# CZY-Code/PHNet

Measured on AMD Instinct MI355X. Metric: clips/s (5x3x320x800) fwd+bwd, higher is better.
Workload: dtype f32 storage / accumulation, every product as an EXACT three-term bf16 split (6 bf16 MFMAs, f32-MFMA accuracy); 1 GPU; 5-frame clip 3x320x800, resnet34 + router + lane head, fwd+bwd+AdamW, 1 clip/GPU/step, random-init weights; parallelism=dp1, launch=hipGraph replay of the whole step

## Files before the change

include/phnet_hip.h:

```cpp
#ifndef PHNET_HIP_H
#define PHNET_HIP_H
#include <stdint.h>
#ifdef __cplusplus
extern "C" {
#endif

#define PHNET_OK 0
#define PHNET_ERR_ARG (-1)
#define PHNET_ERR_WORKSPACE (-2)
#define PHNET_ERR_LAUNCH (-3)
#define PHNET_ABI_VERSION 1

int phnet_abi_version(void);

int phnet_lane_nms(const float* rows, const float* scores, const int32_t* counts, int64_t frames,
                   int64_t k_max, int32_t n_offsets, float thresh, int64_t top_k,
                   int64_t* keep, int64_t* num_to_keep, int64_t* parent, void* stream);

int phnet_lane_decode(const float* lines, int64_t frames, int32_t N, int32_t n_offsets, float conf_thresh,
                      float nms_thresh, int64_t top_k, float img_w, uint8_t* keep_mask, int64_t* num,
                      int64_t* keep_c, int64_t* anchors, int64_t* anchors_sorted, float* kept_rows, void* stream);

int phnet_lane_points(const float* kept_rows, const int64_t* num, const float* prior_ys, int64_t F, int32_t L, int32_t S,
                      float* points, int32_t* count, int32_t* lanes_num, int32_t* slot, void* stream);

int phnet_lane_track(const float* kept_rows, const int64_t* num, int64_t B, int32_t T, int32_t L, int32_t S, int32_t M, float thr,
                     int32_t max_age, int32_t* trk_id, int32_t* trk_missed, int32_t* trk_hits, int32_t* trk_ext, float* trk_x,
                     int32_t* next_id, int32_t* track_id, int32_t* track_hits, void* stream);

int phnet_lane_draw(const float* points, const int32_t* count, const int32_t* lanes_num, const int32_t* slot,
                    const int32_t* track_id, int64_t F, int32_t L, int32_t S, double sx, double sy, double oy,
                    int32_t out_h, int32_t out_w, int32_t lane_width, const uint8_t* src, int32_t src_format,
                    int64_t frame_stride, int32_t pitch, int64_t chroma_offset, const int32_t* csc_host,
                    const uint8_t* palette, int32_t alpha, uint8_t* label_map, uint8_t* overlay, void* stream);

int phnet_lane_targets(const float* points, const int32_t* counts, const int32_t* lanes_num, const double* offsets_ys, float* out,
                       int64_t F, int32_t Lin, int32_t P, int32_t R, int32_t S, double img_h, double img_w, double strip_size,
                       double crop, double src_w, double scale_x, double scale_y, int32_t flip, void* stream);
int phnet_lane_targets_aug(const float* points, const int32_t* counts, const int32_t* lanes_num, const double* offsets_ys, float* out,
                           int64_t F, int32_t Lin, int32_t P, int32_t R, int32_t S, double img_h, double img_w, double strip_size,
                           double crop, double src_w, double scale_x, double scale_y, int32_t flip, const int32_t* flip2,
                           const double* fwd, void* stream);
int phnet_lane_targets_clip(const float* points, const int32_t* counts, const int32_t* lanes_num, const double* offsets_ys, float* out,
                            int64_t F, int32_t Lin, int32_t P, int32_t R, int32_t S, double img_h, double img_w, double strip_size,
                            double crop, double src_w, double scale_x, double scale_y, int32_t flip, const int32_t* flip2,
                            const double* fwd, int32_t clip, int32_t* frag_count, void* stream);

int phnet_roi_pool_fwd(const float* fmap, const float* xs, const float* ys, float* out, float* out_cp,
                       int32_t B, int32_t N, int32_t P, int32_t h, int32_t w, int32_t C, void* stream);
int phnet_roi_pool_bwd(const float* dout, const float* fmap, const float* xs, const float* ys,
                       float* dmap, float* dxs,
                       int32_t B, int32_t N, int32_t P, int32_t h, int32_t w, int32_t C, void* stream);

int phnet_conv2d_fwd(const float* x, const float* w, const float* bias, float* y,
                     int32_t N, int32_t Hi, int32_t Wi, int32_t Ci, int32_t Co, int32_t R, int32_t S,
                     int32_t stride, int32_t pad, int32_t relu, void* workspace, uint64_t ws_bytes, void* stream);
uint64_t phnet_conv2d_stats_blocks(int64_t M, int32_t Co, int32_t K, uint64_t ws_bytes);
int phnet_conv2d_fwd_fused(const float* x, const float* w, const float* bias, const float* addend, float* y, float* stats,
                           int32_t N, int32_t Hi, int32_t Wi, int32_t Ci, int32_t Co, int32_t R, int32_t S,
                           int32_t stride, int32_t pad, int32_t relu, void* workspace, uint64_t ws_bytes, void* stream);
int phnet_conv2d_dgrad(const float* dy, const float* w, const float* addend, float* dx,
                       int32_t N, int32_t Hi, int32_t Wi, int32_t Ci, int32_t Co, int32_t R, int32_t S,
                       int32_t stride, int32_t pad, void* workspace, uint64_t ws_bytes, void* stream);
int phnet_conv3p_applies(int64_t M, int32_t Ca, int32_t Nn);
uint64_t phnet_conv3p_packed_bytes(int32_t Co, int32_t Ci);
int phnet_conv3p_pack(const float* w, void* packed, int32_t Co, int32_t Ci, int32_t dgrad, void* stream);
int phnet_conv3p_pack_jobs(const void* jobs, int32_t njobs, int64_t total, void* stream);
uint64_t phnet_conv3p_stats_blocks(int64_t M, int32_t Ca, int32_t Nn, uint64_t ws_bytes);
int phnet_conv3p_fwd(const float* x, const void* packed, const float* bias, const float* addend, float* y, float* stats,
                     int32_t N, int32_t H, int32_t W, int32_t Ca, int32_t Nn, int32_t relu,
                     void* workspace, uint64_t ws_bytes, void* stream);
int phnet_conv2d_plan(int64_t M, int32_t Co, int32_t K, uint64_t ws_bytes, int32_t* bm, int32_t* bn, int32_t* splits,
                      int32_t* k_tile);
int phnet_conv2d_kernel(int32_t dgrad, int32_t N, int32_t Hi, int32_t Wi, int32_t Ci, int32_t Co, int32_t R, int32_t S,
                        int32_t stride, int32_t pad, uint64_t ws_bytes, char* name, int32_t name_cap, int32_t* splits);
int phnet_conv2d_wgrad_kernel(int32_t N, int32_t Hi, int32_t Wi, int32_t Ci, int32_t Co, int32_t R, int32_t S, int32_t stride,
                              int32_t pad, int32_t has_dbias, uint64_t ws_bytes, char* name, int32_t name_cap, int32_t* splits);
int phnet_linear_bwd_kernel(int32_t M, int32_t K, int32_t N, int32_t has_relu_mask, char* name, int32_t name_cap);
int phnet_conv3p_kernel(int64_t M, int32_t Ca, int32_t Nn, uint64_t ws_bytes, char* name, int32_t name_cap, int32_t* splits);
uint64_t phnet_conv2d_wgrad_workspace(int32_t N, int32_t Hi, int32_t Wi, int32_t Ci, int32_t Co,
                                      int32_t R, int32_t S, int32_t stride, int32_t pad);
int phnet_conv2d_wgrad(const float* dy, const float* x, float* dw, float* dbias,
                       int32_t N, int32_t Hi, int32_t Wi, int32_t Ci, int32_t Co, int32_t R, int32_t S,
                       int32_t stride, int32_t pad, int32_t accumulate, void* workspace, uint64_t ws_bytes, void* stream);
int phnet_linear_bwd_fusable(int64_t M, int64_t K, int64_t N);
int phnet_linear_bwd(const float* dy, const float* x, const float* w, const float* relu_y, float* dx, float* dw, float* dbias,
                     int32_t M, int32_t K, int32_t N, int32_t accumulate, void* stream);
int phnet_nchw3_to_nhwc4(const float* x, float* y, int32_t N, int32_t H, int32_t W, void* stream);
int phnet_pad_channels(const float* src, float* dst, int64_t rows, int32_t cs, int32_t cd, void* stream);

uint64_t phnet_ipc_buffer_bytes(int32_t world, uint64_t max_bytes);
int phnet_ipc_alloc(uint64_t bytes, void** ptr);
int phnet_ipc_free(void* ptr);
int phnet_ipc_get_handle(void* ptr, void* handle64);
int phnet_ipc_open_handle(const void* handle64, void** ptr);
int phnet_ipc_close_handle(void* ptr);
int phnet_oneshot_allreduce(void* data, int32_t count, int32_t dtype, const void* peers, int32_t rank, int32_t world,
                            int32_t cap, void* ctrl, void* stream);

uint64_t phnet_channel_partials_size(int64_t M, int32_t C);
int phnet_bn_fwd_stats(const float* x, int64_t M, int32_t C, float eps, float momentum,
                       const float* gamma, const float* beta, float* running_mean, float* running_var,
                       float* save_mean, float* save_invstd, float* scale, float* shift,
                       float* partial, int32_t training, void* stream);
int phnet_bn_finalize_partials(const float* partial, int64_t nblk, int64_t M, int32_t C, float eps, float momentum,
                               const float* gamma, const float* beta, float* running_mean, float* running_var,
                               float* save_mean, float* save_invstd, float* scale, float* shift, void* stream);
int phnet_bn_apply(const float* x, const float* scale, const float* shift, const float* residual, float* y,
                   int64_t M, int32_t C, int32_t relu, void* stream);
int phnet_bn_bwd(const float* dy, const float* x, const float* y, const float* save_mean,
                 const float* save_invstd, const float* gamma, float* dx, float* dres,
                 float* dgamma, float* dbeta, float* partial, float* c1, float* c2,
                 int64_t M, int32_t C, int32_t relu, int32_t dres_accumulate, int32_t param_accumulate, void* stream);

int phnet_bn_bwd_reduce(const float* dy, const float* x, const float* y, const float* mean, const float* invstd,
                        float* sums, float* partial, float* c1_scratch, float* c2_scratch,
                        int64_t M, int32_t C, int32_t relu, void* stream);
int phnet_bn_bwd_apply(const float* dy, const float* x, const float* y, const float* mean, const float* invstd,
                       const float* gamma, const float* c1, const float* c2, float* dx, float* dres,
                       int64_t M, int32_t C, int32_t relu, int32_t dres_accumulate, void* stream);

int phnet_bn_local_sums(const float* x, int64_t M, int32_t C, float* partial, double* sums, void* stream);
int phnet_bn_partials_to_sums(const float* partial, int64_t nblk, int64_t M, int32_t C, double* sums, void* stream);
int phnet_bn_finalize_sums(const double* sums, int32_t C, float eps, float momentum, const float* gamma, const float* beta,
                           float* running_mean, float* running_var, float* save_mean, float* save_invstd,
                           float* scale, float* shift, void* stream);
int phnet_bn_bwd_apply_sums(const float* dy, const float* x, const float* y, const float* mean, const float* invstd,
                            const float* gamma, const float* sums, const double* count, float* c1, float* c2,
                            float* dx, float* dres, int64_t M, int32_t C, int32_t relu, int32_t dres_accumulate, void* stream);

int phnet_preprocess_u8(const uint8_t* frames, float* out, uint8_t* out_u8,
                        const int32_t* xi, const int16_t* xc, const int32_t* yi, const int16_t* yc,
                        int32_t T, int32_t H0, int32_t W0, int32_t crop_top, int32_t out_h, int32_t out_w, int32_t flip,
                        int32_t layout, const float* mean3_host, const float* std3_host, void* stream);
int phnet_preprocess_yuv(const uint8_t* frames, float* out, uint8_t* out_u8,
                         const int32_t* xi, const int16_t* xc, const int32_t* yi, const int16_t* yc,
                         int32_t T, int32_t H0, int32_t W0, int32_t crop_top, int32_t out_h, int32_t out_w, int32_t flip, int32_t layout,
                         int32_t format, int64_t frame_stride, int32_t pitch, int64_t chroma_offset,
                         const int32_t* csc_host, const float* mean3_host, const float* std3_host, void* stream);

int phnet_augment_u8(const uint8_t* frames, float* out, uint8_t* out_u8, const int32_t* flip2, const double* inv, const int32_t* table,
                     int32_t T, int32_t H, int32_t W, int32_t layout, const float* mean3_host, const float* std3_host, void* stream);

int phnet_augment_stencil_u8(const uint8_t* frames, float* out, uint8_t* out_u8, const int32_t* flip2, const double* inv,
                             const int32_t* table, const int32_t* stencil, uint8_t* staged, int32_t T, int32_t H, int32_t W, int32_t layout,
                             const float* mean3_host, const float* std3_host, void* stream);

int phnet_lane_raster(const int32_t* segs, int64_t n_segs, uint32_t* masks, int32_t n_lanes, int32_t height, int32_t width,
                      int32_t lane_width, void* stream);
int phnet_lane_mask_stats(const uint32_t* masks, int32_t n_lanes, int32_t height, int32_t width, const int32_t* pairs,
                          int32_t n_pairs, int64_t* area, int64_t* inter, void* stream);
int phnet_lane_iou_groups(const uint32_t* masks, int32_t n_lanes, int32_t height, int32_t width, const int32_t* groups,
                          int32_t n_groups, int64_t n_entries, int32_t scale, double eps, double* iou, int64_t* area,
                          void* stream);
// ... 199 lines not shown
```

phnet_amd/build.py:

```python
import glob
import os
import subprocess
import sys

HERE = os.path.dirname(os.path.abspath(__file__))
CSRC = os.path.join(HERE, "csrc")
OBJ = os.path.join(HERE, "lib", "obj")
SO = os.path.join(HERE, "lib", "libphnet_hip.so")
FLAGS = ["--offload-arch=gfx950", "-O3", "-std=c++17", "-fPIC", "-fvisibility=hidden", "-Wall", "-Wno-unused-function"]
EXTRA_FLAGS = {"wgrad3s.hip": ["-fno-slp-vectorize"], "wgrad1s.hip": ["-fno-slp-vectorize"]}


def _hipcc():
    for c in (os.environ.get("HIPCC"), "/opt/rocm/bin/hipcc", "hipcc"):
        if c and (os.path.isabs(c) and os.path.exists(c) or not os.path.isabs(c)):
            return c
    raise RuntimeError("hipcc not found")


def build(force: bool = False, verbose: bool = True) -> str:
    os.makedirs(OBJ, exist_ok=True)
    srcs = sorted(glob.glob(os.path.join(CSRC, "*.hip")))
    hdrs = glob.glob(os.path.join(CSRC, "*.h")) + [os.path.join(os.path.dirname(HERE), "include", "phnet_hip.h")]
    newest_hdr = max([os.path.getmtime(h) for h in hdrs] + [0.0])
    objs, procs = [], []
    for s in srcs:
        o = os.path.join(OBJ, os.path.basename(s)[:-4] + ".o")
        objs.append(o)
        if force or not os.path.exists(o) or os.path.getmtime(o) < max(os.path.getmtime(s), newest_hdr):
            if verbose:
                print("[phnet_amd.build] hipcc", os.path.basename(s), flush=True)
            procs.append((s, subprocess.Popen([_hipcc(), *FLAGS, *EXTRA_FLAGS.get(os.path.basename(s), []), "-c", s, "-o", o])))
    for s, p in procs:
        if p.wait() != 0:
            raise RuntimeError(f"hipcc failed on {s}")
    if procs or not os.path.exists(SO) or any(os.path.getmtime(o) > os.path.getmtime(SO) for o in objs):
        subprocess.check_call([_hipcc(), "--offload-arch=gfx950", "-shared", "-fPIC", "-o", SO, *objs])
    return SO


if __name__ == "__main__":
    print(build(force="--force" in sys.argv))
```

phnet_amd/csrc/conv.hip:

```cpp
#include <cstdio>
#include "conv_igemm.h"
#include "tuning.h"

using namespace igemm;

namespace {

constexpr int T3_AROWS = 66;
template <bool DGRAD>
__global__ __launch_bounds__(THREADS) void conv3x3s1_kernel(
    const float* __restrict__ X, const float* __restrict__ Wt, const float* __restrict__ bias,
    const float* __restrict__ addend, float* __restrict__ out, ConvShape g, int relu, float* __restrict__ stats)
{
    constexpr int APITCH = KContigPlanes<64, 16>::PITCH;
    constexpr int APLANE = T3_AROWS * APITCH, AIMG = 3 * APLANE;
    typedef KContigPlanes<64, 16> BP3C;
    typedef KStridedPlanes<64, 16> BP3S;
    constexpr int BIMG = DGRAD ? BP3S::BYTES : BP3C::BYTES;
    constexpr int BPLANE = DGRAD ? BP3S::PLANE : BP3C::PLANE;
    extern __shared__ __attribute__((aligned(16))) float lds[];
    unsigned char* A3 = reinterpret_cast<unsigned char*>(lds);
    unsigned char* B3 = A3 + 2 * AIMG;
    unsigned char* dump = B3 + 2 * BIMG;

    const int W = g.Wi, H = g.Hi, Ca = g.Ci;
    const int M = g.N * H * W, K = 9 * Ca;
    const int CC = Ca >> 4;
    const int tiles_n = (g.Co + 63) >> 6;
    const unsigned tile = xcd_remap(blockIdx.x, gridDim.x);
    const int m0 = (int)(tile / tiles_n) * 64, n0 = (int)(tile % tiles_n) * 64;
    const int u_begin = blockIdx.z * g.k_per_split, u_end = min(3 * CC, u_begin + g.k_per_split);
    const int tid = threadIdx.x, lane = tid & 63, wave = tid >> 6;
    const int wm = (wave >> 1) * 32, wn = (wave & 1) * 32;

    constexpr unsigned OOB = 0x80000000u;
    __amdgpu_buffer_rsrc_t x_rsrc = __builtin_amdgcn_make_buffer_rsrc((void*)X, 0, (int)min((long)M * Ca * 4, (long)0x7fffffff), 0x00020000);
    __amdgpu_buffer_rsrc_t w_rsrc = __builtin_amdgcn_make_buffer_rsrc((void*)Wt, 0, (int)min((long)g.Co * K * 4, (long)0x7fffffff), 0x00020000);
    int a_off[2], a_ok[2], a_lds[2];
#pragma unroll
    for (int i = 0; i < 2; ++i) {
        const int idx = tid + 256 * i, row = idx >> 2, chunk = idx & 3;
        const bool rowok = idx < 4 * T3_AROWS;
        const int t = m0 - 1 + row;
        const bool tok = rowok && (unsigned)t < (unsigned)M;
        const int tt = tok ? t : 0;
        const int y = (tt / W) % H;
        a_ok[i] = (tok && y >= 1 ? 1 : 0) | (tok ? 2 : 0) | (tok && y + 1 < H ? 4 : 0);
        a_off[i] = (t * Ca + chunk * 4) * 4;
        a_lds[i] = rowok ? row * APITCH + chunk * 8 : -1;
    }
    const int a_row = tid >> 2, a_chunk = tid & 3;
    const int b_kk = tid >> 4, b_ch = tid & 15;
    int b_off, b_lds;
    if (!DGRAD) {
        const int n = n0 + a_row;
        b_off = n < g.Co ? (n * K + a_chunk * 4) * 4 : (int)OOB;
        b_lds = a_row * BP3C::PITCH + a_chunk * 8;
    } else {
        const int n = n0 + b_ch * 4;
        b_off = n < g.Co ? (b_kk * 9 * g.Co + n) * 4 : (int)OOB;
        b_lds = b_kk * BP3S::PITCH + b_ch * 8;
    }
    int la_dy = u_begin / CC, la_cc = u_begin - la_dy * CC, la_u = u_begin;
    int lb_dy = la_dy, lb_cc = la_cc, lb_u = u_begin, lb_dx = 0;
    const bool wave0 = __builtin_amdgcn_readfirstlane(wave) == 0;
    auto load_a = [&](f32x4 (&reg)[2]) {
        const bool uok = la_u < u_end;
        const int s_a = ((la_dy - 1) * W * Ca + la_cc * 16) * 4;
        {
            const bool ok = uok && ((a_ok[0] >> la_dy) & 1);
            reg[0] = __builtin_bit_cast(f32x4, __builtin_amdgcn_raw_buffer_load_b128(x_rsrc, ok ? a_off[0] + s_a : (int)OOB, 0, 0));
        }
        if (wave0) {
            const bool ok = uok && ((a_ok[1] >> la_dy) & 1);
            reg[1] = __builtin_bit_cast(f32x4, __builtin_amdgcn_raw_buffer_load_b128(x_rsrc, ok ? a_off[1] + s_a : (int)OOB, 0, 0));
        }
        ++la_u; ++la_cc;
        const int wrap = la_cc == CC;
        la_cc = wrap ? 0 : la_cc;
        la_dy += wrap;
    };
    auto load_b = [&](f32x4& reg) {
        const bool uok = lb_u < u_end;
        const int s_b = !DGRAD ? ((lb_dy * 3 + lb_dx) * Ca + lb_cc * 16) * 4
                               : ((lb_cc * 16 * 3 + (2 - lb_dy)) * 3 + (2 - lb_dx)) * g.Co * 4;
// ... 195 lines not shown
    const int mma = tuning().mma_mode;
    if (mma == 3 && M <= 2048) return {64, 64};
    if (mma >= 1) {
        if (N >= 128 && ceil_div64(M, 128) * ceil_div64(N, 128) >= 300) return {128, 128};
        if (ceil_div64(M, 128) * ceil_div64(N, 64) >= 1250) return {128, 64};
    }
    return {64, 64};
}

struct ConvPlan { int bm, bn, splits; long tiles; };

int k_tile_for(long M, int K, int ci, int bm, int bn)
{
    const int mma = tuning().mma_mode;
    if (M <= (mma == 3 ? 256 : 2048) && K >= 64) return (mma == 3 && tuning().deep_kt3 == 32) ? 32 : 64;
    if (mma == 3) return BK;
    if (mma >= 1 && bm == 64 && bn == 64 && ci % 32 == 0) return 32;
    return BK;
}

ConvPlan plan_conv(long M, int Co, int K, bool has_ws, size_t ws_bytes)
{
    const Tuning& tn = tuning();
    TileChoice t = pick_tile(M, Co);
    if (tn.force_bm) {
        t = {tn.force_bm, tn.force_bn};
        ConvPlan f{t.bm, t.bn, 1, ceil_div64(M, t.bm) * ceil_div64(Co, t.bn)};
        int splits = tn.force_splits > 0 ? tn.force_splits : 1;
        while (splits > 1 && (!has_ws || (size_t)splits * M * Co * sizeof(float) > ws_bytes)) --splits;
        f.splits = splits;
        return f;
    }
    ConvPlan p{t.bm, t.bn, 1, ceil_div64(M, t.bm) * ceil_div64(Co, t.bn)};
    const bool deep = M <= (tn.mma_mode == 3 ? 256 : 2048) && K >= 64;
    if (has_ws && p.tiles < (deep ? 400 : 900)) {
        int splits = (int)min((long)8, max((long)1, (1250 + p.tiles / 2) / p.tiles));
        while (splits > 1 && K / splits < 256) --splits;
        while (splits > 1 && (size_t)splits * M * Co * sizeof(float) > ws_bytes) --splits;
        p.splits = splits;
    }
    return p;
}

ConvPick pick_conv(const ConvShape& g, bool dgrad, bool has_ws, size_t ws_bytes)
{
    const Tuning& tn = tuning();
    const long M = (long)g.N * g.Ho * g.Wo;
    const int K = g.R * g.S * g.Ci;
    const ConvPlan t = plan_conv(M, g.Co, K, has_ws, ws_bytes);
    ConvPick p{};
    p.dgrad = dgrad; p.bm = t.bm; p.bn = t.bn; p.splits = t.splits; p.tiles = t.tiles;
    p.bkt = tn.force_kt ? tn.force_kt : k_tile_for(M, K, g.Ci, t.bm, t.bn);
    p.mma = tn.mma_mode;
    p.pf = p.mma == 3 ? ((tn.pf == 4 || tn.pf == 2) ? tn.pf : 1) : (p.mma == 0 && tn.pf == 4) ? 4 : 1;
    const bool uni = (g.Ci % p.bkt) == 0 && tn.uniform_tap;
    p.uni = uni && t.bm == 64 && t.bn == 64;
    p.buf = p.uni && g.in_dil == 1 && tn.buf_loads && p.mma == 3;
    p.taps3 = tn.taps3 && p.buf && g.R == 3 && g.S == 3 && g.stride == 1 && g.pad == 1 && g.Ho == g.Hi && g.Wo == g.Wi &&
              p.bkt == 16 && p.pf == 4 && g.Wi >= 2 && M * (long)g.Ci * 4 < 0x7fffffffL && (long)g.Co * K * 4 < 0x7fffffffL;
    return p;
}

int conv_kernel_name(const ConvPick& p, char* name, int cap)
{
    static const char* const tf[2] = {"false", "true"};
    const int n = p.taps3 ? snprintf(name, (size_t)cap, "conv3x3s1_kernel<%s>", tf[p.dgrad])
                          : snprintf(name, (size_t)cap, "conv_igemm_kernel<%d, %d, %s, %d, %s, %d, %d, %s>", p.bm, p.bn, tf[p.dgrad], p.bkt,
                                     tf[p.uni], p.mma, p.pf, tf[p.buf]);
    return n < cap ? PHNET_OK : PHNET_ERR_ARG;
}

#define PHNET_LAUNCH_CONV___(DGRAD_, BM_, BN_, BKT_, UNI_, PF_)                                                         \
    do {                                                                                                                \
        if (p.buf) PHNET_LAUNCH_CONV____(DGRAD_, BM_, BN_, BKT_, UNI_, 3, PF_, UNI_);                                   \
        else PHNET_LAUNCH_CONV____(DGRAD_, BM_, BN_, BKT_, UNI_, 3, PF_, false);                                        \
    } while (0)
#define PHNET_LAUNCH_CONV_(DGRAD_, BM_, BN_, BKT_, UNI_)                                                                \
    do {                                                                                                                \
        if (p.pf == 4) PHNET_LAUNCH_CONV___(DGRAD_, BM_, BN_, BKT_, UNI_, 4);                                           \
        else if (p.pf == 2) PHNET_LAUNCH_CONV___(DGRAD_, BM_, BN_, BKT_, UNI_, 2);                                      \
        else PHNET_LAUNCH_CONV___(DGRAD_, BM_, BN_, BKT_, UNI_, 1);                                                     \
    } while (0)

template <bool DGRAD>
int launch_conv(const float* X, const float* W, const float* bias, const float* addend, float* out, float* workspace,
                size_t ws_bytes, ConvShape g, int relu, hipStream_t st, float* stats = nullptr)
{
    const ConvPick p = pick_conv(g, DGRAD, workspace != nullptr, ws_bytes);
    const long M = (long)g.N * g.Ho * g.Wo;
    const int K = g.R * g.S * g.Ci;
    const int splits = p.splits;
    g.splits = splits;
    float* dst = splits > 1 ? workspace : out;
    dim3 grid((unsigned)p.tiles, 1, (unsigned)splits);
    const int ksteps = (K + p.bkt - 1) / p.bkt;
    g.k_per_split = ((ksteps + splits - 1) / splits) * p.bkt;
    if (p.taps3) {
        const int units = 3 * (g.Ci / 16);
        g.k_per_split = (units + splits - 1) / splits;
        constexpr size_t lds_ = 2 * 3 * T3_AROWS * KContigPlanes<64, 16>::PITCH +
                                2 * (size_t)(DGRAD ? KStridedPlanes<64, 16>::BYTES : KContigPlanes<64, 16>::BYTES) + 3 * 512;
        hipLaunchKernelGGL((conv3x3s1_kernel<DGRAD>), grid, dim3(THREADS), lds_, st,
                           X, W, bias, addend, dst, g, relu, splits > 1 ? (float*)nullptr : stats);
    } else {
        const ConvLaunch a{X, W, bias, addend, dst, splits > 1 ? (float*)nullptr : stats, &g, relu, grid, st};
        if (p.mma != 3) launch_conv_alt(p, a);
        else PHNET_LAUNCH_CONV_TILES(DGRAD);
    }
    if (splits > 1) {
        const long total4 = M * g.Co / 4;
        hipLaunchKernelGGL(splitk_reduce_kernel, dim3((unsigned)ceil_div64(total4, 256)), dim3(256), 0, st,
                           workspace, out, bias, addend, total4, g.Co, splits, relu, 0, stats);
    }
    return phnet_launch_status();
}

}

PHNET_API int phnet_conv2d_plan(int64_t M, int32_t Co, int32_t K, uint64_t ws_bytes, int32_t* bm, int32_t* bn, int32_t* splits,
                                int32_t* k_tile)
{
    ConvShape g;
    if (M < 1 || M > 0x7fffffffL || Co < 1 || K < 1 || !bm || !bn || !splits || !k_tile) return PHNET_ERR_ARG;
    fwd_shape((int)M, 1, 1, K, Co, 1, 1, 1, 0, &g);
    const ConvPick p = pick_conv(g, false, ws_bytes > 0, (size_t)ws_bytes);
    *bm = p.bm; *bn = p.bn; *splits = p.splits; *k_tile = p.bkt;
    return PHNET_OK;
}

PHNET_API int phnet_conv2d_kernel(int32_t dgrad, int32_t N, int32_t Hi, int32_t Wi, int32_t Ci, int32_t Co, int32_t R, int32_t S,
                                  int32_t stride, int32_t pad, uint64_t ws_bytes, char* name, int32_t name_cap, int32_t* splits)
{
    ConvShape g;
    if (!conv_args_ok(N, Hi, Wi, Ci, Co, R, S, stride, pad) || N < 1 || !name || name_cap < 1 || !splits) return PHNET_ERR_ARG;
    if (dgrad ? (stride > 2 || !dgrad_shape(N, Hi, Wi, Ci, Co, R, S, stride, pad, &g)) : !fwd_shape(N, Hi, Wi, Ci, Co, R, S, stride, pad, &g))
        return PHNET_ERR_ARG;
    const ConvPick p = pick_conv(g, dgrad != 0, ws_bytes > 0, (size_t)ws_bytes);
    *splits = p.splits;
    return conv_kernel_name(p, name, name_cap);
}

PHNET_API int phnet_conv2d_fwd(const float* x, const float* w, const float* bias, float* y,
                               int32_t N, int32_t Hi, int32_t Wi, int32_t Ci, int32_t Co, int32_t R, int32_t S,
                               int32_t stride, int32_t pad, int32_t relu,
                               void* workspace, uint64_t ws_bytes, void* stream)
{
    ConvShape g;
    if (!conv_args_ok(N, Hi, Wi, Ci, Co, R, S, stride, pad)) return PHNET_ERR_ARG;
    if (N == 0) return PHNET_OK;
    if (!x || !w || !y || !fwd_shape(N, Hi, Wi, Ci, Co, R, S, stride, pad, &g)) return PHNET_ERR_ARG;
    return launch_conv<false>(x, w, bias, nullptr, y, (float*)workspace, ws_bytes, g, relu, (hipStream_t)stream);
}

static long conv_stats_blocks(long M, int Co, int K, bool has_ws, size_t ws_bytes)
{
    const ConvPlan t = plan_conv(M, Co, K, has_ws, ws_bytes);
    return t.splits > 1 ? ceil_div64(M * Co / 4, 256) : t.tiles / ceil_div64(Co, t.bn) * (t.bm / 32);
}

PHNET_API uint64_t phnet_conv2d_stats_blocks(int64_t M, int32_t Co, int32_t K, uint64_t ws_bytes)
{
    if (M < 1 || Co < 4 || K < 1) return 0;
    return (uint64_t)conv_stats_blocks((long)M, Co, K, ws_bytes > 0, (size_t)ws_bytes);
}

PHNET_API int phnet_conv2d_fwd_fused(const float* x, const float* w, const float* bias, const float* addend, float* y, float* stats,
                                     int32_t N, int32_t Hi, int32_t Wi, int32_t Ci, int32_t Co, int32_t R, int32_t S,
                                     int32_t stride, int32_t pad, int32_t relu,
                                     void* workspace, uint64_t ws_bytes, void* stream)
{
    ConvShape g;
    if (!conv_args_ok(N, Hi, Wi, Ci, Co, R, S, stride, pad)) return PHNET_ERR_ARG;
    if (stats && (bias || addend || relu || (Co & (Co - 1)) || Co > 1024)) return PHNET_ERR_ARG;
    if (N == 0) return PHNET_OK;
    if (!x || !w || !y || !fwd_shape(N, Hi, Wi, Ci, Co, R, S, stride, pad, &g)) return PHNET_ERR_ARG;
    return launch_conv<false>(x, w, bias, addend, y, (float*)workspace, ws_bytes, g, relu, (hipStream_t)stream, stats);
}

PHNET_API int phnet_conv2d_dgrad(const float* dy, const float* w, const float* addend, float* dx,
                                 int32_t N, int32_t Hi, int32_t Wi, int32_t Ci, int32_t Co, int32_t R, int32_t S,
                                 int32_t stride, int32_t pad, void* workspace, uint64_t ws_bytes, void* stream)
{
    ConvShape g;
    if (!conv_args_ok(N, Hi, Wi, Ci, Co, R, S, stride, pad)) return PHNET_ERR_ARG;
    if (stride > 2) return PHNET_ERR_ARG;
    if (N == 0) return PHNET_OK;
    if (!dy || !w || !dx || !dgrad_shape(N, Hi, Wi, Ci, Co, R, S, stride, pad, &g)) return PHNET_ERR_ARG;
    return launch_conv<true>(dy, w, nullptr, addend, dx, (float*)workspace, ws_bytes, g, 0, (hipStream_t)stream);
}

PHNET_API int phnet_nchw3_to_nhwc4(const float* x, float* y, int32_t N, int32_t H, int32_t W, void* stream)
{
    if (N < 0 || H < 1 || W < 1) return PHNET_ERR_ARG;
    if (N == 0) return PHNET_OK;
    if (!x || !y) return PHNET_ERR_ARG;
    const long total = (long)N * H * W;
    hipLaunchKernelGGL(nchw3_to_nhwc4_kernel, dim3((unsigned)ceil_div64(total, 256)), dim3(256), 0, (hipStream_t)stream,
                       x, y, N, H * W);
    return phnet_launch_status();
}

// ... 10 lines not shown
```

phnet_amd/csrc/tuning.h:

```cpp
#pragma once

struct Tuning {
    int mma_mode = 3;
    int pf = 4;
    int buf_loads = 1;
    int uniform_tap = 1;
    int taps3 = 1;
    int deep_kt3 = 64;
    int force_bm = 0, force_bn = 0, force_splits = 0;
    int force_kt = 0;
    int wgrad_bm128 = 1;
    int wgrad_smallp = 1;
    int wgrad_bkw = 16;
    int wgrad3 = 1;
    int wgrad3_bkw = 16;
    int wgrad3s = 1;
    int wgrad1s = 1;
    int wgrad_target = 768;
    int wgrad3_target = 256;
    int smallp_max_tiles = 400;
    int p3_target = 512;
    int p3_wide = 1;
    int gate_wave = 1;
    int dyn_mfma = 1;
    int dyn_rows = 1;
};

Tuning& tuning();
```

phnet_amd/csrc/tuning.hip:

```cpp
#include "common.h"
#include "tuning.h"

Tuning& tuning() { static Tuning t; return t; }

PHNET_API int phnet_tune_reset(void) { tuning() = Tuning{}; return PHNET_OK; }
PHNET_API int phnet_tune_mma_get(void) { return tuning().mma_mode; }

PHNET_API int phnet_tune_force_conv_tile(int32_t bm, int32_t bn, int32_t splits)
{
    if (bm != 0 && !((bm == 64 || bm == 128) && (bn == 64 || bn == 128))) return PHNET_ERR_ARG;
    Tuning& t = tuning();
    t.force_bm = bm; t.force_bn = bn; t.force_splits = splits;
    return PHNET_OK;
}

PHNET_API int phnet_tune_force_k_tile(int32_t kt)
{
    Tuning& t = tuning();
    if (kt == -1 || kt == -2) { t.uniform_tap = kt == -2; return PHNET_OK; }
    if (kt == -5 || kt == -6) { t.taps3 = kt == -6; return PHNET_OK; }
    if (kt == -32 || kt == -64) { t.deep_kt3 = -kt; return PHNET_OK; }
    if (kt == -101 || kt == -102 || kt == -104) { t.pf = -kt - 100; return PHNET_OK; }
    if (kt == -200 || kt == -201) { t.buf_loads = -kt - 200; return PHNET_OK; }
    if (kt != 0 && kt != 16 && kt != 32 && kt != 64) return PHNET_ERR_ARG;
    t.force_kt = kt;
    return PHNET_OK;
}

PHNET_API int phnet_tune_wgrad(int32_t allow_bm128, int32_t target_blocks)
{
    if (target_blocks == 0 || target_blocks < -1024) return PHNET_ERR_ARG;
    Tuning& t = tuning();
    t.wgrad_bm128 = allow_bm128 & 1; t.wgrad_smallp = !(allow_bm128 & 2); t.wgrad_bkw = (allow_bm128 & 4) ? 32 : 16;
    t.wgrad3 = !(allow_bm128 & 8); t.wgrad3_bkw = (allow_bm128 & 16) ? 32 : 16;
    t.wgrad3s = !(allow_bm128 & 32); t.wgrad1s = !(allow_bm128 & 64);
    (target_blocks < 0 ? t.wgrad3_target : t.wgrad_target) = target_blocks < 0 ? -target_blocks : target_blocks;
    return PHNET_OK;
}

PHNET_API int phnet_tune_mma(int32_t mode)
{
    if (mode < 0 || mode > 3) return PHNET_ERR_ARG;
    tuning().mma_mode = mode;
    tuning().pf = mode == 3 ? 4 : 1;
    return PHNET_OK;
}

PHNET_API int phnet_conv3p_tune(int32_t target_workgroups)
{
    if (target_workgroups == -1 || target_workgroups == -2) { tuning().p3_wide = target_workgroups == -2; return PHNET_OK; }
    if (target_workgroups < 1) return PHNET_ERR_ARG;
    tuning().p3_target = target_workgroups;
    return PHNET_OK;
}

PHNET_API int phnet_tune_gate_wave(int32_t on) { tuning().gate_wave = on != 0; return PHNET_OK; }
PHNET_API int phnet_tune_dyn_mfma(int32_t on) { tuning().dyn_mfma = (on & 1) != 0; tuning().dyn_rows = !(on & 2); return PHNET_OK; }
```

phnet_amd/hip_ops.py:

```python
import ctypes
import os
from typing import Optional, Tuple

import torch

from ._lib import check, lib

_WS = {}

TIMER = None


def _kernel(query, *shape_args, has_splits=True):
    name, splits = ctypes.create_string_buffer(96), ctypes.c_int32(0)
    check(query(*shape_args, name, len(name), *([ctypes.byref(splits)] if has_splits else [])), "kernel query")
    return name.value.decode(), splits.value


def _timed_launch(sym_fn, flops, launch, shape=None, nbytes=None):
    if TIMER is None:
        return launch()
    sym, splits = sym_fn()
    e0, e1 = torch.cuda.Event(enable_timing=True), torch.cuda.Event(enable_timing=True)
    e0.record()
# ... 148 lines not shown
            for dg in kinds:
                ca, nn = (co, ci) if dg else (ci, co)
                assert ca % 16 == 0 and nn % 32 == 0, w.shape
                img = self.buf[off:off + nbytes]
                rows.append([int(w.data_ptr()), int(img.data_ptr()), co | (ci << 32), int(dg), first])
                first += 9 * (ca // 16) * (nn // 32) * 64
                off += nbytes
                per[dg] = img
            self.images.append(per)
        self.total = first
        self.jobs = torch.tensor(rows, dtype=torch.int64).to(dev)

    def matches(self, weights) -> bool:
        return self.ptrs == tuple(int(w.data_ptr()) for w in weights)

    def refresh(self):
        check(lib().phnet_conv3p_pack_jobs(_ptr(self.jobs), self.jobs.shape[0], self.total, _stream()), "phnet_conv3p_pack_jobs")


def conv3p(x: torch.Tensor, packed: torch.Tensor, nn: int, dgrad: bool = False, bias=None, addend=None, relu: bool = False,
           stats: bool = False):
    _req(x, name="x")
    n, h, w_, ca = x.shape
    out = torch.empty((n, h, w_, nn), dtype=torch.float32, device=x.device)
    m = n * h * w_
    need = 8 * m * nn * 4 if m * nn < (1 << 23) else 0
    ws = workspace(need, x.device) if need else None
    part, nblk = None, 0
    if stats:
        nblk = int(lib().phnet_conv3p_stats_blocks(m, ca, nn, need))
        part = workspace(nblk * 2 * nn * 4, x.device, 1)
    if addend is not None:
        _req(addend, name="addend")
        assert addend.shape == out.shape
    _timed_launch(lambda: _kernel(lib().phnet_conv3p_kernel, m, ca, nn, need),
                  2.0 * m * nn * 9 * ca,
                  lambda: check(lib().phnet_conv3p_fwd(_ptr(x), _ptr(packed), _ptr(bias), _ptr(addend), _ptr(out), _ptr(part), n, h, w_, ca, nn,
                                                       int(relu), _ptr(ws), need, _stream()), "phnet_conv3p_fwd"),
                  shape=("dgrad" if dgrad else "fwd", m, nn, 9 * ca, 3),
                  nbytes=4.0 * m * (ca + nn) + 6.0 * 9 * ca * nn + (4.0 * m * nn if addend is not None else 0.0))
    return (out, (part, nblk)) if stats else out


def conv2d_dgrad(dy, w, in_hw: Tuple[int, int], stride: int, pad: int, addend: Optional[torch.Tensor] = None,
                 out: Optional[torch.Tensor] = None):
    _req(dy, name="dy"); _req(w, name="w")
    n = dy.shape[0]
    co, r, s, ci = w.shape
    hi, wi = in_hw
    dx = torch.empty((n, hi, wi, ci), dtype=torch.float32, device=dy.device) if out is None else _req(out, name="out")
    assert dx.shape == (n, hi, wi, ci)
    need = 8 * n * hi * wi * ci * 4 if n * hi * wi * ci < (1 << 23) else 0
    ws = workspace(need, dy.device) if need else None
    m, k = n * hi * wi, r * s * co
    _timed_launch(lambda: _kernel(lib().phnet_conv2d_kernel, 1, n, hi, wi, ci, co, r, s, stride, pad, need), 2.0 * dy.shape[0] * dy.shape[1] * dy.shape[2] * co * r * s * ci,
                  lambda: check(lib().phnet_conv2d_dgrad(_ptr(dy), _ptr(w), _ptr(addend), _ptr(dx), n, hi, wi, ci, co, r, s, stride,
                                                         pad, _ptr(ws), need, _stream()), "phnet_conv2d_dgrad"),
                  shape=("dgrad", m, ci, k, r), nbytes=4.0 * (dy.numel() + m * ci + co * r * s * ci))
    return dx


CONV3P = os.environ.get("PHNET_CONV3P", "1") != "0"


def conv2d_wgrad(dy, x, w_shape, stride: int, pad: int, dw: Optional[torch.Tensor] = None, accumulate: bool = False,
                 dbias: Optional[torch.Tensor] = None):
    _req(dy, name="dy"); _req(x, name="x")
    n, hi, wi, ci = x.shape
    co, r, s, _ = w_shape
    if dw is None:
        dw = torch.empty((co, r, s, ci), dtype=torch.float32, device=x.device)
        assert not accumulate
    need = lib().phnet_conv2d_wgrad_workspace(n, hi, wi, ci, co, r, s, stride, pad)
    ws = workspace(need, x.device) if need else None
    ho, wo = conv_out_hw(hi, wi, r, s, stride, pad)
    _timed_launch(lambda: _kernel(lib().phnet_conv2d_wgrad_kernel, n, hi, wi, ci, co, r, s, stride, pad, int(dbias is not None), need),
                  2.0 * n * ho * wo * co * r * s * ci,
                  lambda: check(lib().phnet_conv2d_wgrad(_ptr(dy), _ptr(x), _ptr(dw), _ptr(dbias), n, hi, wi, ci, co, r, s, stride,
                                                         pad, int(accumulate), _ptr(ws), need, _stream()), "phnet_conv2d_wgrad"),
                  shape=("wgrad", co, r * s * ci, n * ho * wo, r), nbytes=4.0 * (dy.numel() + x.numel() + co * r * s * ci))
    return dw


def linear_fwd(x2d, w, bias, relu: bool = False):
    m, k = x2d.shape
    return conv2d_fwd(x2d.view(m, 1, 1, k), w.view(w.shape[0], 1, 1, k), bias, 1, 0, relu).view(m, w.shape[0])


def linear_dgrad(dy2d, w):
    m, n = dy2d.shape
    k = w.shape[1]
    return conv2d_dgrad(dy2d.view(m, 1, 1, n), w.view(n, 1, 1, k), (1, 1), 1, 0).view(m, k)


def linear_wgrad(dy2d, x2d, dw: Optional[torch.Tensor] = None, accumulate: bool = False, dbias: Optional[torch.Tensor] = None):
    m, n = dy2d.shape
    k = x2d.shape[1]
    out = conv2d_wgrad(dy2d.view(m, 1, 1, n), x2d.view(m, 1, 1, k), (n, 1, 1, k), 1, 0,
                       None if dw is None else dw.view(n, 1, 1, k), accumulate, dbias)
    return out.view(n, k)


def linear_bwd_fusable(m: int, k: int, n: int) -> bool:
    return bool(lib().phnet_linear_bwd_fusable(m, k, n))


def linear_bwd(dy2d, x2d, w, dw: torch.Tensor, dbias: Optional[torch.Tensor], accumulate: bool, relu_y: Optional[torch.Tensor] = None):
    _req(dy2d, name="dy"); _req(x2d, name="x"); _req(w, name="w"); _req(dw, name="dw")
    m, n = dy2d.shape
    k = x2d.shape[1]
    dx = torch.empty((m, k), dtype=torch.float32, device=dy2d.device)
    _timed_launch(lambda: _kernel(lib().phnet_linear_bwd_kernel, m, k, n, int(relu_y is not None), has_splits=False), 4.0 * m * n * k,
                  lambda: check(lib().phnet_linear_bwd(_ptr(dy2d), _ptr(x2d), _ptr(w), _ptr(relu_y), _ptr(dx), _ptr(dw), _ptr(dbias), m, k, n,
                                                       int(accumulate), _stream()), "phnet_linear_bwd"), shape=("linbwd", m, n, k, 1))
    return dx


def nchw3_to_nhwc4(x):
    _req(x, name="frames")
    n, c, h, w = x.shape
    assert c == 3
    y = torch.empty((n, h, w, 4), dtype=torch.float32, device=x.device)
    check(lib().phnet_nchw3_to_nhwc4(_ptr(x), _ptr(y), n, h, w, _stream()), "phnet_nchw3_to_nhwc4")
    return y


def pad_channels(src2d, cd: int):
    _req(src2d, name="src")
    rows, cs = src2d.shape
    dst = torch.empty((rows, cd), dtype=torch.float32, device=src2d.device)
    check(lib().phnet_pad_channels(_ptr(src2d), _ptr(dst), rows, cs, cd, _stream()), "phnet_pad_channels")
    return dst


def _partials(m, c, device, slot=1):
    nfloats = lib().phnet_channel_partials_size(m, c)
    return workspace(nfloats * 4, device, slot)


def bn_fwd(x, gamma, beta, running_mean, running_var, training: bool, eps: float, momentum: float,
           residual=None, relu: bool = True, partials=None):
    _req(x, name="x")
    c = x.shape[-1]
    m = x.numel() // c
    dev = x.device
    scale = torch.empty(c, dtype=torch.float32, device=dev)
    shift = torch.empty(c, dtype=torch.float32, device=dev)
    sm = torch.empty(c, dtype=torch.float32, device=dev) if training else None
    si = torch.empty(c, dtype=torch.float32, device=dev) if training else None
    if training and partials is not None:
        check(lib().phnet_bn_finalize_partials(_ptr(partials[0]), int(partials[1]), m, c, eps, momentum, _ptr(gamma), _ptr(beta),
                                               _ptr(running_mean), _ptr(running_var), _ptr(sm), _ptr(si), _ptr(scale), _ptr(shift),
                                               _stream()), "phnet_bn_finalize_partials")
    else:
        part = _partials(m, c, dev) if training else None
        check(lib().phnet_bn_fwd_stats(_ptr(x), m, c, eps, momentum, _ptr(gamma), _ptr(beta), _ptr(running_mean),
                                       _ptr(running_var), _ptr(sm), _ptr(si), _ptr(scale), _ptr(shift), _ptr(part),
                                       int(training), _stream()), "phnet_bn_fwd_stats")
    y = torch.empty_like(x)
    check(lib().phnet_bn_apply(_ptr(x), _ptr(scale), _ptr(shift), _ptr(residual), _ptr(y), m, c, int(relu), _stream()),
          "phnet_bn_apply")
    return y, sm, si


def bn_bwd(dy, x, y, save_mean, save_invstd, gamma, relu: bool, dres: Optional[torch.Tensor] = None,
           dres_accumulate: bool = False, dgamma: Optional[torch.Tensor] = None, dbeta: Optional[torch.Tensor] = None,
           param_accumulate: bool = False):
    _req(dy, name="dy")
    c = x.shape[-1]
    m = x.numel() // c
    dev = x.device
    dx = torch.empty_like(x)
    dgamma = torch.empty(c, dtype=torch.float32, device=dev) if dgamma is None else dgamma
    dbeta = torch.empty(c, dtype=torch.float32, device=dev) if dbeta is None else dbeta
# ... 1216 lines not shown
```

Baseline: 66.92 clips/s.

## Add warp-specialized producer/consumer GEMM kernel for mid-size linear fwd and dgrad

Adds a new linear-layer GEMM kernel in which dedicated producer waves stream A/B tiles through a register ring into double-buffered LDS with the three-term bf16 split. Consumer waves run the MFMA chains on those tiles. It is used for linear forward and dgrad when M is 257-2048, K is at least 1024 and N is a multiple of 128, and only when the planned workgroup count nearly fills the 256 CUs. It reuses the existing split-K planner and reduce kernel. The aim is to overlap global loads with MFMA work on these mid-size linears, at the cost of a second kernel family and extra launch-planning logic.

```diff
diff --git a/include/phnet_hip.h b/include/phnet_hip.h
--- a/include/phnet_hip.h
+++ b/include/phnet_hip.h
@@ -70,6 +70,13 @@
 int phnet_conv3p_fwd(const float* x, const void* packed, const float* bias, const float* addend, float* y, float* stats,
                      int32_t N, int32_t H, int32_t W, int32_t Ca, int32_t Nn, int32_t relu,
                      void* workspace, uint64_t ws_bytes, void* stream);
+int phnet_linrows_applies(int64_t M, int32_t K, int32_t N, int32_t dgrad);
+int phnet_linrows_fwd(const float* x, const float* w, const float* bias, float* y, int64_t M, int32_t K, int32_t N, int32_t relu,
+                      void* workspace, uint64_t ws_bytes, void* stream);
+int phnet_linrows_dgrad(const float* dy, const float* w, float* dx, int64_t M, int32_t K, int32_t N, void* workspace,
+                        uint64_t ws_bytes, void* stream);
+int phnet_linrows_kernel(int64_t M, int32_t K, int32_t N, int32_t dgrad, uint64_t ws_bytes, char* name, int32_t name_cap,
+                         int32_t* splits);
 int phnet_conv2d_plan(int64_t M, int32_t Co, int32_t K, uint64_t ws_bytes, int32_t* bm, int32_t* bn, int32_t* splits,
                       int32_t* k_tile);
 int phnet_conv2d_kernel(int32_t dgrad, int32_t N, int32_t Hi, int32_t Wi, int32_t Ci, int32_t Co, int32_t R, int32_t S,
diff --git a/phnet_amd/build.py b/phnet_amd/build.py
--- a/phnet_amd/build.py
+++ b/phnet_amd/build.py
@@ -8,7 +8,7 @@
 OBJ = os.path.join(HERE, "lib", "obj")
 SO = os.path.join(HERE, "lib", "libphnet_hip.so")
 FLAGS = ["--offload-arch=gfx950", "-O3", "-std=c++17", "-fPIC", "-fvisibility=hidden", "-Wall", "-Wno-unused-function"]
-EXTRA_FLAGS = {"wgrad3s.hip": ["-fno-slp-vectorize"], "wgrad1s.hip": ["-fno-slp-vectorize"]}
+EXTRA_FLAGS = {"wgrad3s.hip": ["-fno-slp-vectorize"], "wgrad1s.hip": ["-fno-slp-vectorize"], "linrows.hip": ["-fno-slp-vectorize"]}
 
 
 def _hipcc():
diff --git a/phnet_amd/csrc/conv.hip b/phnet_amd/csrc/conv.hip
--- a/phnet_amd/csrc/conv.hip
+++ b/phnet_amd/csrc/conv.hip
@@ -1,6 +1,7 @@
 #include <cstdio>
 #include "conv_igemm.h"
 #include "tuning.h"
+#include "linrows.h"
 
 using namespace igemm;
 
@@ -362,6 +363,12 @@
         else PHNET_LAUNCH_CONV___(DGRAD_, BM_, BN_, BKT_, UNI_, 1);                                                     \
     } while (0)
 
+int k_per_split_of(const ConvPick& p, int K)
+{
+    const int ksteps = (K + p.bkt - 1) / p.bkt;
+    return ((ksteps + p.splits - 1) / p.splits) * p.bkt;
+}
+
 template <bool DGRAD>
 int launch_conv(const float* X, const float* W, const float* bias, const float* addend, float* out, float* workspace,
                 size_t ws_bytes, ConvShape g, int relu, hipStream_t st, float* stats = nullptr)
@@ -373,8 +380,7 @@
     g.splits = splits;
     float* dst = splits > 1 ? workspace : out;
     dim3 grid((unsigned)p.tiles, 1, (unsigned)splits);
-    const int ksteps = (K + p.bkt - 1) / p.bkt;
-    g.k_per_split = ((ksteps + splits - 1) / splits) * p.bkt;
+    g.k_per_split = k_per_split_of(p, K);
     if (p.taps3) {
         const int units = 3 * (g.Ci / 16);
         g.k_per_split = (units + splits - 1) / splits;
@@ -397,6 +403,22 @@
 
 }
 
+ConvSplit phnet_linear_split(long M, int K, int N, bool dgrad, bool has_ws, size_t ws_bytes)
+{
+    ConvShape g;
+    if (dgrad) dgrad_shape((int)M, 1, 1, N, K, 1, 1, 1, 0, &g);
+    else fwd_shape((int)M, 1, 1, K, N, 1, 1, 1, 0, &g);
+    const ConvPick p = pick_conv(g, dgrad, has_ws, ws_bytes);
+    return ConvSplit{p.splits, k_per_split_of(p, K)};
+}
+
+void phnet_splitk_reduce(const float* part, float* out, const float* bias, long M, int N, int splits, int relu, hipStream_t st)
+{
+    const long total4 = M * N / 4;
+    hipLaunchKernelGGL(splitk_reduce_kernel, dim3((unsigned)ceil_div64(total4, 256)), dim3(256), 0, st,
+                       part, out, bias, (const float*)nullptr, total4, N, splits, relu, 0, (float*)nullptr);
+}
+
 PHNET_API int phnet_conv2d_plan(int64_t M, int32_t Co, int32_t K, uint64_t ws_bytes, int32_t* bm, int32_t* bn, int32_t* splits,
                                 int32_t* k_tile)
 {
diff --git a/phnet_amd/csrc/linrows.h b/phnet_amd/csrc/linrows.h
--- /dev/null
+++ b/phnet_amd/csrc/linrows.h
@@ -0,0 +1,8 @@
+#pragma once
+#include "common.h"
+
+struct ConvSplit { int splits, k_per_split; };
+
+ConvSplit phnet_linear_split(long M, int K, int N, bool dgrad, bool has_ws, size_t ws_bytes);
+
+void phnet_splitk_reduce(const float* part, float* out, const float* bias, long M, int N, int splits, int relu, hipStream_t st);
diff --git a/phnet_amd/csrc/linrows.hip b/phnet_amd/csrc/linrows.hip
--- /dev/null
+++ b/phnet_amd/csrc/linrows.hip
@@ -0,0 +1,254 @@
+#include <cstdio>
+#include <type_traits>
+#include "conv_common.h"
+#include "linrows.h"
+#include "tuning.h"
+
+using namespace igemm;
+
+namespace {
+
+constexpr int R_FM = 5;
+constexpr int R_TN = 128;
+constexpr int R_PRODUCERS = 4;
+constexpr int R_CUS = 256;
+
+struct RowsShape {
+    int M, K, N;
+    int splits, k_per_split;
+    int tiles_m;
+};
+
+template <bool DGRAD, int WM> struct RowsCfg {
+    static constexpr int TM = WM * R_FM * 32;
+    static constexpr int CONSUMERS = 4 * WM;
+    static constexpr int NT = (CONSUMERS + R_PRODUCERS) * 64;
+    static constexpr int A_LOADS = (TM * 4 + R_PRODUCERS * 64 - 1) / (R_PRODUCERS * 64);
+    static constexpr int A_ROWS = A_LOADS * 64;
+    static constexpr int B_LOADS = 2;
+    static constexpr int PF = WM == 2 ? 3 : 4;
+    typedef KContigPlanes<A_ROWS, BK> AP;
+    typedef KContigPlanes<R_TN, BK> BPC;
+    typedef KStridedPlanes<R_TN, BK> BPS;
+    static constexpr int B_PITCH = DGRAD ? BPS::PITCH : BPC::PITCH;
+    static constexpr int B_PLANE = DGRAD ? BPS::PLANE : BPC::PLANE;
+    static constexpr int STAGE = AP::BYTES + 3 * B_PLANE;
+    static constexpr int LDS = 2 * STAGE;
+};
+
+template <bool DGRAD, int WM>
+__global__ __launch_bounds__((RowsCfg<DGRAD, WM>::NT)) void linrows_kernel(const float* __restrict__ A, const float* __restrict__ W,
+                                                                         const float* __restrict__ bias, float* __restrict__ out,
+                                                                         RowsShape g, int relu)
+{
+    typedef RowsCfg<DGRAD, WM> C;
+    typedef typename C::AP AP;
+    extern __shared__ __attribute__((aligned(16))) unsigned char lds_raw[];
+    const int M = g.M, K = g.K, N = g.N;
+    const unsigned tile = xcd_remap(blockIdx.x, gridDim.x);
+    const int m0 = (int)(tile % g.tiles_m) * C::TM, n0 = (int)(tile / g.tiles_m) * R_TN;
+    const int k_begin = blockIdx.z * g.k_per_split, k_end = min(K, k_begin + g.k_per_split);
+    const int nsteps = k_begin < k_end ? (k_end - k_begin) / BK : 0;
+    const int tid = threadIdx.x, lane = tid & 63;
+    const int wave = __builtin_amdgcn_readfirstlane(tid >> 6);
+    const bool final_pass = g.splits == 1;
+
+    if (wave >= C::CONSUMERS) {
+        if (nsteps == 0) return;
+        const int p = tid - C::CONSUMERS * 64;
+        const int a_row = p >> 2, a_chunk = p & 3;
+        constexpr unsigned OOB = 0x80000000u;
+        __amdgpu_buffer_rsrc_t rsrc_a = __builtin_amdgcn_make_buffer_rsrc((void*)A, 0, (int)min((long)M * K * 4, (long)0x7fffffff), 0x00020000);
+        __amdgpu_buffer_rsrc_t rsrc_b = __builtin_amdgcn_make_buffer_rsrc((void*)W, 0, (int)min((long)N * K * 4, (long)0x7fffffff), 0x00020000);
+        int a_off[C::A_LOADS], a_lds[C::A_LOADS], b_off[C::B_LOADS], b_lds[C::B_LOADS];
+#pragma unroll
+        for (int i = 0; i < C::A_LOADS; ++i) {
+            const int row = a_row + 64 * i, m = m0 + row;
+            a_off[i] = (row < C::TM && m < M) ? (m * K + a_chunk * 4) * 4 : (int)OOB;
+            a_lds[i] = row * AP::PITCH + a_chunk * 8;
+        }
+#pragma unroll
+        for (int i = 0; i < C::B_LOADS; ++i) {
+            if (!DGRAD) {
+                const int n = n0 + a_row + 64 * i;
+                b_off[i] = n < N ? (n * K + a_chunk * 4) * 4 : (int)OOB;
+                b_lds[i] = (a_row + 64 * i) * C::B_PITCH + a_chunk * 8;
+            } else {
+                const int idx = p + 256 * i, kk = idx >> 5, ch = idx & 31, n = n0 + ch * 4;
+                b_off[i] = n < N ? (kk * N + n) * 4 : (int)OOB;
+                b_lds[i] = kk * C::B_PITCH + ch * 8;
+            }
+        }
+        constexpr int NL = C::A_LOADS + C::B_LOADS;
+        f32x4 ring[C::PF][NL];
+        int ld = 0;
+        auto load_step = [&](f32x4 (&reg)[NL]) {
+            const bool ok = ld < nsteps;
+            const int s_a = (k_begin + BK * ld) * 4;
+            const int s_b = DGRAD ? (k_begin + BK * ld) * N * 4 : s_a;
+#pragma unroll
+            for (int i = 0; i < C::A_LOADS; ++i)
+                reg[i] = __builtin_bit_cast(f32x4, __builtin_amdgcn_raw_buffer_load_b128(rsrc_a, ok ? a_off[i] + s_a : (int)OOB, 0, 0));
+#pragma unroll
+            for (int i = 0; i < C::B_LOADS; ++i)
+                reg[C::A_LOADS + i] = __builtin_bit_cast(f32x4, __builtin_amdgcn_raw_buffer_load_b128(rsrc_b, ok ? b_off[i] + s_b : (int)OOB, 0, 0));
+            ++ld;
+        };
+        auto store_step = [&](int buf_off, const f32x4 (&reg)[NL]) {
+#pragma unroll
+            for (int i = 0; i < C::A_LOADS; ++i) store_split3<AP::PLANE>(lds_raw + buf_off, a_lds[i], reg[i]);
+#pragma unroll
+            for (int i = 0; i < C::B_LOADS; ++i) store_split3<C::B_PLANE>(lds_raw + buf_off + AP::BYTES, b_lds[i], reg[C::A_LOADS + i]);
+        };
+#pragma unroll
+        for (int d = 0; d < C::PF; ++d) load_step(ring[d]);
+        store_step(0, ring[0]);
+        load_step(ring[0]);
+        __syncthreads();
+        int o_st = C::STAGE;
+        bool reload = true;
+        auto body = [&](auto U, int) {
+            constexpr int slot = (decltype(U)::value + 1) % C::PF;
+            store_step(o_st, ring[slot]);
+            if (reload) load_step(ring[slot]);
+            __syncthreads();
+            o_st = C::STAGE - o_st;
+        };
+        int t = 0;
+        for (; t + C::PF <= nsteps; t += C::PF) unroll_iterations<C::PF>(body, t);
+        reload = false;
+        tail_iterations<C::PF - 1>(body, t, nsteps);
+        return;
+    }
+
+    const int wm = (wave >> 2) * (R_FM * 32), wn = (wave & 3) * 32;
+    const int n = n0 + wn + frag_col(lane);
+    const bool nok = n < N;
+    f32x16 acc[R_FM][1];
+    {
+        const float bv = (final_pass && bias && nok) ? bias[n] : 0.f;
+#pragma unroll
+        for (int f = 0; f < R_FM; ++f)
+#pragma unroll
+            for (int e = 0; e < 16; ++e) acc[f][0][e] = bv + 0.f;
+    }
+    if (nsteps > 0) {
+        const unsigned char* a_src = lds_raw + wm * AP::PITCH;
+        const unsigned char* b_src = lds_raw + AP::BYTES + (DGRAD ? wn * 2 : wn * C::B_PITCH);
+        int o = 0;
+        __syncthreads();
+        for (int t = 0; t < nsteps; ++t) {
+            Frag3 fa[R_FM], fb[1];
+            if (!DGRAD) read_kcontig3<1, C::B_PITCH, C::B_PLANE>(b_src + o, lane, 0, fb);
+            else read_kstrided3<1, C::B_PITCH, C::B_PLANE>(b_src + o, lane, 0, fb);
+            read_kcontig3<R_FM, AP::PITCH, AP::PLANE>(a_src + o, lane, 0, fa);
+            mma3_step<R_FM, 1>(fa, fb, acc);
+            __syncthreads();
+            o = C::STAGE - o;
+        }
+    }
+    float* dst = out + (size_t)blockIdx.z * M * N;
+    if (nok) {
+#pragma unroll
+        for (int f = 0; f < R_FM; ++f)
+#pragma unroll
+            for (int e = 0; e < 16; ++e) {
+                const int m = m0 + wm + 32 * f + frag_row(lane, e);
+                if (m < M) dst[(size_t)m * N + n] = (final_pass && relu) ? fmaxf(acc[f][0][e], 0.f) : acc[f][0][e];
+            }
+    }
+}
+
+inline long cdiv(long a, long b) { return (a + b - 1) / b; }
+
+bool rows_ok(long M, int K, int N)
+{
+    return tuning().mma_mode == 3 && M >= 1 && K >= BK && (K % BK) == 0 && N >= 4 && (N & 3) == 0 &&
+           (M + 320) * K * 4 < 0x7fffffffL && (long)N * K * 4 < 0x7fffffffL && (M + 320) * N * 4 < 0x7fffffffL;
+}
+
+struct RowsPlan { int wm, splits, k_per_split; long tiles_m, tiles_n; };
+
+RowsPlan rows_plan(long M, int K, int N, bool dgrad, size_t ws_bytes)
+{
+    const ConvSplit s = phnet_linear_split(M, K, N, dgrad, ws_bytes > 0, ws_bytes);
+    RowsPlan p;
+    p.splits = s.splits;
+    p.k_per_split = s.k_per_split;
+    p.wm = s.splits == 1 ? 2 : 1;
+    p.tiles_m = cdiv(M, p.wm * R_FM * 32);
+    p.tiles_n = cdiv(N, R_TN);
+    return p;
+}
+
+bool rows_applies(long M, int K, int N, bool dgrad)
+{
+    const Tuning& tn = tuning();
+    if (!tn.linrows || tn.force_bm || tn.force_kt || !rows_ok(M, K, N)) return false;
+    if (M <= 256 || M > 2048 || (N % R_TN) != 0 || K < 1024) return false;
+    const size_t ws_bytes = M * N < (1L << 23) ? (size_t)8 * M * N * 4 : 0;
+    const RowsPlan p = rows_plan(M, K, N, dgrad, ws_bytes);
+    const long wgs = p.tiles_m * p.tiles_n * p.splits;
+    return wgs > R_CUS * 3 / 4 && wgs <= R_CUS;
+}
+
+int rows_kernel_name(const RowsPlan& p, bool dgrad, char* name, int cap)
+{
+    return snprintf(name, (size_t)cap, "linrows_kernel<%s, %d>", dgrad ? "true" : "false", p.wm) < cap ? PHNET_OK : PHNET_ERR_ARG;
+}
+
+template <bool DGRAD, int WM>
+bool launch_rows_as(const float* a, const float* w, const float* bias, float* dst, const RowsShape& g, int relu, dim3 grid, hipStream_t st)
+{
+    typedef RowsCfg<DGRAD, WM> C;
+    static bool attr = false;
+    if (!attr && !(attr = phnet_allow_dynamic_lds({(const void*)linrows_kernel<DGRAD, WM>}, C::LDS))) return false;
+    hipLaunchKernelGGL((linrows_kernel<DGRAD, WM>), grid, dim3(C::NT), C::LDS, st, a, w, bias, dst, g, relu);
+    return true;
+}
+
+template <bool DGRAD>
+int launch_rows(const float* a, const float* w, const float* bias, float* out, long M, int K, int N, int relu, float* workspace,
+                size_t ws_bytes, hipStream_t st)
+{
+    const RowsPlan p = rows_plan(M, K, N, DGRAD, workspace ? ws_bytes : 0);
+    const RowsShape g{(int)M, K, N, p.splits, p.k_per_split, (int)p.tiles_m};
+    float* dst = p.splits > 1 ? workspace : out;
+    const dim3 grid((unsigned)(p.tiles_m * p.tiles_n), 1, (unsigned)p.splits);
+    if (!(p.wm == 2 ? launch_rows_as<DGRAD, 2>(a, w, bias, dst, g, relu, grid, st) : launch_rows_as<DGRAD, 1>(a, w, bias, dst, g, relu, grid, st)))
+        return PHNET_ERR_LAUNCH;
+    if (p.splits > 1) phnet_splitk_reduce(workspace, out, bias, M, N, p.splits, relu, st);
+    return phnet_launch_status();
+}
+
+}
+
+PHNET_API int phnet_linrows_applies(int64_t M, int32_t K, int32_t N, int32_t dgrad)
+{
+    return rows_applies((long)M, K, N, dgrad != 0) ? 1 : 0;
+}
+
+PHNET_API int phnet_linrows_kernel(int64_t M, int32_t K, int32_t N, int32_t dgrad, uint64_t ws_bytes, char* name, int32_t name_cap,
+                                   int32_t* splits)
+{
+    if (!rows_ok((long)M, K, N) || !name || name_cap < 1 || !splits) return PHNET_ERR_ARG;
+    const RowsPlan p = rows_plan((long)M, K, N, dgrad != 0, (size_t)ws_bytes);
+    *splits = p.splits;
+    return rows_kernel_name(p, dgrad != 0, name, name_cap);
+}
+
+PHNET_API int phnet_linrows_fwd(const float* x, const float* w, const float* bias, float* y, int64_t M, int32_t K, int32_t N,
+                                int32_t relu, void* workspace, uint64_t ws_bytes, void* stream)
+{
+    if (M == 0) return PHNET_OK;
+    if (!x || !w || !y || !rows_ok((long)M, K, N)) return PHNET_ERR_ARG;
+    return launch_rows<false>(x, w, bias, y, (long)M, K, N, relu, (float*)workspace, (size_t)ws_bytes, (hipStream_t)stream);
+}
+
+PHNET_API int phnet_linrows_dgrad(const float* dy, const float* w, float* dx, int64_t M, int32_t K, int32_t N, void* workspace,
+                                  uint64_t ws_bytes, void* stream)
+{
+    if (M == 0) return PHNET_OK;
+    if (!dy || !w || !dx || !rows_ok((long)M, K, N)) return PHNET_ERR_ARG;
+    return launch_rows<true>(dy, w, nullptr, dx, (long)M, K, N, 0, (float*)workspace, (size_t)ws_bytes, (hipStream_t)stream);
+}
diff --git a/phnet_amd/csrc/tuning.h b/phnet_amd/csrc/tuning.h
--- a/phnet_amd/csrc/tuning.h
+++ b/phnet_amd/csrc/tuning.h
@@ -6,6 +6,7 @@
     int buf_loads = 1;
     int uniform_tap = 1;
     int taps3 = 1;
+    int linrows = 1;
     int deep_kt3 = 64;
     int force_bm = 0, force_bn = 0, force_splits = 0;
     int force_kt = 0;
diff --git a/phnet_amd/csrc/tuning.hip b/phnet_amd/csrc/tuning.hip
--- a/phnet_amd/csrc/tuning.hip
+++ b/phnet_amd/csrc/tuning.hip
@@ -22,6 +22,7 @@
     if (kt == -32 || kt == -64) { t.deep_kt3 = -kt; return PHNET_OK; }
     if (kt == -101 || kt == -102 || kt == -104) { t.pf = -kt - 100; return PHNET_OK; }
     if (kt == -200 || kt == -201) { t.buf_loads = -kt - 200; return PHNET_OK; }
+    if (kt == -300 || kt == -301) { t.linrows = -kt - 300; return PHNET_OK; }
     if (kt != 0 && kt != 16 && kt != 32 && kt != 64) return PHNET_ERR_ARG;
     t.force_kt = kt;
     return PHNET_OK;
diff --git a/phnet_amd/hip_ops.py b/phnet_amd/hip_ops.py
--- a/phnet_amd/hip_ops.py
+++ b/phnet_amd/hip_ops.py
@@ -254,14 +254,39 @@
     return dw
 
 
+def linrows_applies(m: int, k: int, n: int, dgrad: bool) -> bool:
+    return bool(lib().phnet_linrows_applies(int(m), int(k), int(n), int(dgrad)))
+
+
+def _linrows(dgrad: bool, a2d, w, bias, relu: bool, n: int):
+    _req(a2d, name="x"); _req(w, name="w")
+    m, k = a2d.shape
+    out = torch.empty((m, n), dtype=torch.float32, device=a2d.device)
+    need = 8 * m * n * 4 if m * n < (1 << 23) else 0
+    ws = workspace(need, a2d.device) if need else None
+    if dgrad:
+        launch = lambda: check(lib().phnet_linrows_dgrad(_ptr(a2d), _ptr(w), _ptr(out), m, k, n, _ptr(ws), need, _stream()),
+                               "phnet_linrows_dgrad")
+    else:
+        launch = lambda: check(lib().phnet_linrows_fwd(_ptr(a2d), _ptr(w), _ptr(bias), _ptr(out), m, k, n, int(relu), _ptr(ws), need,
+                                                       _stream()), "phnet_linrows_fwd")
+    _timed_launch(lambda: _kernel(lib().phnet_linrows_kernel, m, k, n, int(dgrad), need), 2.0 * m * n * k, launch,
+                  shape=("dgrad" if dgrad else "fwd", m, n, k, 1), nbytes=4.0 * (m * k + m * n + n * k))
+    return out
+
+
 def linear_fwd(x2d, w, bias, relu: bool = False):
     m, k = x2d.shape
+    if linrows_applies(m, k, w.shape[0], False):
+        return _linrows(False, x2d, w, bias, relu, w.shape[0])
     return conv2d_fwd(x2d.view(m, 1, 1, k), w.view(w.shape[0], 1, 1, k), bias, 1, 0, relu).view(m, w.shape[0])
 
 
 def linear_dgrad(dy2d, w):
     m, n = dy2d.shape
     k = w.shape[1]
+    if linrows_applies(m, n, k, True):
+        return _linrows(True, dy2d, w, None, False, k)
     return conv2d_dgrad(dy2d.view(m, 1, 1, n), w.view(n, 1, 1, k), (1, 1), 1, 0).view(m, k)
 
 
```

New measurement: 68.50 clips/s (median of 6 runs). +2.4%, better.
